# linnanwang/FastGen

Hardware: AMD Instinct MI355X
Metric: images/sec at 4-step distilled (DMD2) sampling (higher is better)
Workload: dtype fp32 (tensors, accumulate) with split-bf16 x3 MFMA conv products; 1 GPU; EDM CIFAR-10 32x32 SongUNet (55.7M params) DMD2 4-step 'sde' sampling, batch=512 per GPU; global_batch=512, sample_steps=4, parallelism=replicas x1 (no data-path collective), graph=True

## Files before the change

### fastgen_amd/csrc/conv.h

```cpp
#pragma once
#include <hip/hip_runtime.h>

struct ConvArgs {
    const void* src1;
    const void* src2;
    int C1, C2;
    int Hs, Ws;
    int H, W;
    int B;
    const float2* ab;
    const void* wpack;
    const void* wpack_ws;
    const float* bias;
    const float* temb;
    int temb_stride;
    const void* resid;
    float scale;
    void* out;
    int Cout;
    float2* stats;
    int dbg;
    void* q_out;
    void* k_out;
    void* vt_out;
    const float* gate = nullptr;
    int gate_stride = 0;
    int act = 0;
    int heads = 0, head_dim = 0;
    size_t heads_lo_off = 0;
};

enum { PRO_NONE = 0, PRO_GN = 1, PRO_GN_SILU = 2 };
enum { RES_NONE = 0, RES_DOWN = 1, RES_UP = 2 };
enum { OUT_NHWC = 0, OUT_QKV = 1, OUT_TOK = 2, OUT_HEADS = 3 };

int launch_conv_fused(int dtype, int ks, int pro, int res, int outmode, const ConvArgs& a, hipStream_t stream);
int conv_stat_slots(int W);
bool conv_ws_supported(int dtype, int ks, int pro, int res, int outmode, const ConvArgs& a);
bool conv_ws_enabled();
int launch_conv_ws(int res, const ConvArgs& a, hipStream_t stream, bool prepare_only, int pro = PRO_GN_SILU);
bool conv_ws_shape_ok(int dtype, int cout, int cin, int res);
int launch_pack_conv_weights_ws(const float* w_oihw, void* wpack_ws, int cout, int cin, hipStream_t stream);
bool conv_x3ws_supported(int ks, int pro, int res, int outmode, const ConvArgs& a);
bool conv_x3ws_shape_ok(int cout, int cin, int res);
int conv_x3ws_stat_slots(int W);
int launch_conv_x3ws(int res, const ConvArgs& a, hipStream_t stream, bool prepare_only, int pro = PRO_GN_SILU);
int launch_pack_conv_weights_x3ws(const float* w_oihw, void* wpack_ws, int cout, int cin, hipStream_t stream);
int conv_launch_stat_slots(int dtype, int ks, int pro, int res, int outmode, const ConvArgs& a);
int launch_conv_ws_debug(const ConvArgs& a, int abl, hipStream_t stream);
int launch_conv_debug(int dtype, const ConvArgs& a, hipStream_t stream);
int conv_prepare_all(int dtype);
size_t conv_pack_elems(int cout, int cin, int ks);
int launch_pack_conv_weights(int dtype, const float* w_oihw, void* wpack, int cout, int cin, int ks, int qkv_perm,
                             hipStream_t stream);
```

### fastgen_amd/csrc/conv.hip

```cpp
#include "common.h"
#include "conv.h"
#include <stdlib.h>

#include <type_traits>

namespace {

constexpr int PITCH = 144;
constexpr int NTHR = 256;

template <int KS, int LOGW>
struct Geom {
    static constexpr int W = 1 << LOGW;
    static constexpr int LOGTW = (LOGW == 5) ? 4 : LOGW;
    static constexpr int TW = 1 << LOGTW;
    static constexpr int LOGTH = 3;
    static constexpr int TH = 1 << LOGTH;
    static constexpr int IMGS = 128 / (TH * TW);
    static constexpr int TCOLS = W / TW;
    static constexpr int TPI = (IMGS > 1) ? 1 : (W / TH) * TCOLS;
    static constexpr int PAD = KS / 2;
    static constexpr int HW_ = TW + 2 * PAD;
    static constexpr int HH_ = TH + 2 * PAD;
    static constexpr int HALO_PIX = IMGS * HH_ * HW_;
// ... 427 lines not shown
                for (int i4 = 0; i4 < 16; i4 += 4) {
                    const int p = mt * 32 + acc_row(i4, h);
                    const int x = col0 + (p & (G::TW - 1));
                    const int y = row0 + ((p >> G::LOGTW) & (G::TH - 1));
                    const int n = n_base + (p >> (G::LOGTW + G::LOGTH));
                    if (n < a.B)
                    {
                        const size_t vo = ((size_t)n * (OUTMODE == OUT_HEADS ? a.heads * a.head_dim : 256) + cl) * HWo + y * G::W + x;
                        const f32x4 vv = {acc[mt][nt][i4] + bias, acc[mt][nt][i4 + 1] + bias, acc[mt][nt][i4 + 2] + bias,
                                          acc[mt][nt][i4 + 3] + bias};
                        if constexpr (OUTMODE == OUT_HEADS && std::is_same<T, bf16x3>::value)
                            store4_split(reinterpret_cast<__bf16*>(vt) + vo, a.heads_lo_off, vv);
                        else
                            store4(vt + vo, vv);
                    }
                }
            }
        }
    }
}

template <typename T>
__global__ void pack_conv_weights_kernel(const float* __restrict__ w, typename DT<T>::WT* __restrict__ out, int cout, int cin, int ks,
                                         int qkv_perm) {
    constexpr int KC = DT<T>::KC, KK = KC / 16, WP = DT<T>::WPARTS;
    const int taps = ks * ks;
    const size_t total = (size_t)cout * cin * taps;
    for (size_t idx = (size_t)blockIdx.x * blockDim.x + threadIdx.x; idx < total; idx += (size_t)gridDim.x * blockDim.x) {
        size_t t = idx;
        const int j = t % 8; t /= 8;
        const int lane = t % 64; t /= 64;
        const int kk = t % KK; t /= KK;
        const int tap = t % taps; t /= taps;
        const int nchunk = cin / KC;
        const int chunk = t % nchunk; t /= nchunk;
        const int nt = (int)t;
        int co = nt * 32 + (lane & 31);
        if (qkv_perm) {
            const int C = cout / 3;
            co = (co % C) * 3 + co / C;
        }
        const int ci = chunk * KC + kk * 16 + 8 * (lane >> 5) + j;
        const float v = w[((size_t)co * cin + ci) * taps + tap];
        if constexpr (WP == 1) {
            out[idx] = (typename DT<T>::WT)v;
        } else {
            const size_t o = (idx / 512) * 1024 + (idx % 512);
            const __bf16 hi = (__bf16)v;
            out[o] = hi;
            out[o + 512] = (__bf16)(v - (float)hi);
        }
    }
}

size_t g_debug_extra_lds = 0;
bool g_prepare_only = false;

template <typename T, int KS, int PRO, int RES, int LOGW, int OUTMODE, int ABL = 0>
int launch_one(const ConvArgs& a, hipStream_t stream) {
    using G = Geom<KS, LOGW>;
    const int tiles = (G::IMGS > 1) ? (a.B + G::IMGS - 1) / G::IMGS : a.B * G::TPI;
    const size_t lds = 2 * (size_t)G::ABUF + (ABL ? g_debug_extra_lds : 0);
    auto kern = conv_fused_kernel<T, KS, PRO, RES, LOGW, OUTMODE, ABL>;
    static bool attr_done[16] = {};
    const int dev = fg_device_slot();
    if (dev < 0) return (int)hipErrorInvalidDevice;
    if (!attr_done[dev] || (ABL && g_debug_extra_lds)) {
        hipError_t e = hipFuncSetAttribute(reinterpret_cast<const void*>(kern), hipFuncAttributeMaxDynamicSharedMemorySize, (int)lds);
        if (e != hipSuccess) return (int)e;
        attr_done[dev] = true;
    }
    if (g_prepare_only) return 0;
    constexpr int NCOL = 128 * conv_nt(KS, LOGW, OUTMODE);
    dim3 grid(tiles, (a.Cout + NCOL - 1) / NCOL);
    hipLaunchKernelGGL(kern, grid, dim3(NTHR), lds, stream, a);
    return (int)hipGetLastError();
}

template <typename T, int KS, int PRO, int RES, int OUTMODE>
int launch_w(const ConvArgs& a, hipStream_t s) {
    switch (a.W) {
        case 32: return launch_one<T, KS, PRO, RES, 5, OUTMODE>(a, s);
        case 16: return launch_one<T, KS, PRO, RES, 4, OUTMODE>(a, s);
        case 8: return launch_one<T, KS, PRO, RES, 3, OUTMODE>(a, s);
    }
    return (int)hipErrorInvalidValue;
}

template <typename T>
int launch_t(int ks, int pro, int res, int outmode, const ConvArgs& a, hipStream_t s) {
    if (outmode == OUT_QKV) {
        if (ks == 1 && pro == PRO_GN && res == RES_NONE) return launch_w<T, 1, PRO_GN, RES_NONE, OUT_QKV>(a, s);
        return (int)hipErrorInvalidValue;
    }
    if (outmode == OUT_TOK || outmode == OUT_HEADS) {
        if (ks != 1 || pro != PRO_NONE || res != RES_NONE || a.W != 16) return (int)hipErrorInvalidValue;
        return outmode == OUT_TOK ? launch_one<T, 1, PRO_NONE, RES_NONE, 4, OUT_TOK>(a, s) : launch_one<T, 1, PRO_NONE, RES_NONE, 4, OUT_HEADS>(a, s);
    }
    if (ks == 3 && pro == PRO_GN_SILU) {
        if (res == RES_NONE) return launch_w<T, 3, PRO_GN_SILU, RES_NONE, OUT_NHWC>(a, s);
        if (res == RES_UP) return launch_w<T, 3, PRO_GN_SILU, RES_UP, OUT_NHWC>(a, s);
    }
    if (ks == 3 && pro == PRO_NONE && res == RES_NONE) return launch_w<T, 3, PRO_NONE, RES_NONE, OUT_NHWC>(a, s);
    if (ks == 1 && pro == PRO_NONE) {
        if (res == RES_NONE) return launch_w<T, 1, PRO_NONE, RES_NONE, OUT_NHWC>(a, s);
        if (res == RES_DOWN) return launch_w<T, 1, PRO_NONE, RES_DOWN, OUT_NHWC>(a, s);
        if (res == RES_UP) return launch_w<T, 1, PRO_NONE, RES_UP, OUT_NHWC>(a, s);
    }
    return (int)hipErrorInvalidValue;
}

int dispatch_t(int dtype, int ks, int pro, int res, int outmode, const ConvArgs& a, hipStream_t s) {
    switch (dtype) {
        case 0: return launch_t<float>(ks, pro, res, outmode, a, s);
        case 1: return launch_t<__bf16>(ks, pro, res, outmode, a, s);
        case 2: return launch_t<bf16x3>(ks, pro, res, outmode, a, s);
    }
    return (int)hipErrorInvalidValue;
}

}

int launch_conv_debug(int dtype, const ConvArgs& a, hipStream_t stream) {
    if (dtype != 1 || a.W != 32) return (int)hipErrorInvalidValue;
    g_debug_extra_lds = (a.dbg & 16) ? 48 * 1024 : 0;
    switch (a.dbg & 15) {
        case 0: return launch_one<__bf16, 3, PRO_GN_SILU, RES_NONE, 5, OUT_NHWC, 0>(a, stream);
        case 1: return launch_one<__bf16, 3, PRO_GN_SILU, RES_NONE, 5, OUT_NHWC, 1>(a, stream);
        case 2: return launch_one<__bf16, 3, PRO_GN_SILU, RES_NONE, 5, OUT_NHWC, 2>(a, stream);
        case 3: return launch_one<__bf16, 3, PRO_GN_SILU, RES_NONE, 5, OUT_NHWC, 3>(a, stream);
        case 4: return launch_one<__bf16, 3, PRO_GN_SILU, RES_NONE, 5, OUT_NHWC, 4>(a, stream);
        case 5: return launch_one<__bf16, 3, PRO_GN_SILU, RES_NONE, 5, OUT_NHWC, 5>(a, stream);
        case 6: return launch_one<__bf16, 3, PRO_GN_SILU, RES_NONE, 5, OUT_NHWC, 6>(a, stream);
        case 7: return launch_one<__bf16, 3, PRO_GN_SILU, RES_NONE, 5, OUT_NHWC, 7>(a, stream);
    }
    return (int)hipErrorInvalidValue;
}

int launch_conv_fused(int dtype, int ks, int pro, int res, int outmode, const ConvArgs& a, hipStream_t stream) {
    const int kc = dtype == 1 ? DT<__bf16>::KC : DT<float>::KC;
    if (a.H != a.W || (a.W != 8 && a.W != 16 && a.W != 32)) return (int)hipErrorInvalidValue;
    const bool tok = outmode == OUT_TOK || outmode == OUT_HEADS;
    if ((a.C1 % kc) || (a.C2 % kc) || (a.Cout % (tok ? 64 : 256)) || a.B <= 0) return (int)hipErrorInvalidValue;
    if (outmode == OUT_HEADS && (a.heads <= 0 || (a.head_dim % 4) || a.Cout != 3 * a.heads * a.head_dim || ((a.heads * a.head_dim) % 64) ||
                                 !a.q_out || !a.k_out || !a.vt_out))
        return (int)hipErrorInvalidValue;
    if (res == RES_NONE && (a.Hs != a.H || a.Ws != a.W)) return (int)hipErrorInvalidValue;
    if (res == RES_DOWN && (a.Hs != 2 * a.H || a.Ws != 2 * a.W)) return (int)hipErrorInvalidValue;
    if (res == RES_UP && (2 * a.Hs != a.H || 2 * a.Ws != a.W)) return (int)hipErrorInvalidValue;
    if (pro != PRO_NONE && !a.ab) return (int)hipErrorInvalidValue;
    if (outmode == OUT_QKV && (a.Cout != 768 || a.W > 16)) return (int)hipErrorInvalidValue;
    if (conv_ws_enabled() && conv_ws_supported(dtype, ks, pro, res, outmode, a)) return launch_conv_ws(res, a, stream, false, pro);
    if (dtype == 2 && conv_ws_enabled() && conv_x3ws_supported(ks, pro, res, outmode, a)) return launch_conv_x3ws(res, a, stream, false, pro);
    return dispatch_t(dtype, ks, pro, res, outmode, a, stream);
}

bool conv_ws_enabled() {
    static const bool on = [] {
        const char* e = getenv("FASTGEN_AMD_CONV_WS");
        return !(e && e[0] == '0');
    }();
    return on;
}

int conv_launch_stat_slots(int dtype, int ks, int pro, int res, int outmode, const ConvArgs& a) {
    if (dtype == 2 && conv_ws_enabled() && conv_x3ws_supported(ks, pro, res, outmode, a)) return conv_x3ws_stat_slots(a.W);
    return conv_stat_slots(a.W);
}

int conv_stat_slots(int W) { return W == 32 ? Geom<3, 5>::TPI : (W == 16 ? Geom<3, 4>::TPI : Geom<3, 3>::TPI); }

int conv_prepare_all(int dtype) {
    g_prepare_only = true;
    int rc = 0;
    ConvArgs a{};
    a.B = 1;
    a.Cout = 256;
    const int ws[3] = {8, 16, 32};
    for (int wi = 0; wi < 3 && !rc; ++wi) {
        a.W = a.H = ws[wi];
        for (int res = 0; res < 3 && !rc; ++res) {
            if (res != RES_DOWN)
                rc = dispatch_t(dtype, 3, PRO_GN_SILU, res, OUT_NHWC, a, nullptr);
            if (!rc) rc = dispatch_t(dtype, 1, PRO_NONE, res, OUT_NHWC, a, nullptr);
        }
        if (!rc) rc = dispatch_t(dtype, 3, PRO_NONE, RES_NONE, OUT_NHWC, a, nullptr);
        if (!rc && a.W <= 16) rc = dispatch_t(dtype, 1, PRO_GN, RES_NONE, OUT_QKV, a, nullptr);
        if (!rc && a.W == 16) rc = dispatch_t(dtype, 1, PRO_NONE, RES_NONE, OUT_TOK, a, nullptr);
        if (!rc && a.W == 16) rc = dispatch_t(dtype, 1, PRO_NONE, RES_NONE, OUT_HEADS, a, nullptr);
    }
    g_prepare_only = false;
    if (!rc && dtype == 2) {
        ConvArgs w{};
        for (int res : {RES_NONE, RES_UP})
            for (int ww : {32, 16, 8}) {
                if (ww == 8 && res != RES_NONE) continue;
                w.W = w.H = ww;
                if (!rc) rc = launch_conv_x3ws(res, w, nullptr, true, PRO_GN_SILU);
                if (!rc && res == RES_NONE) rc = launch_conv_x3ws(res, w, nullptr, true, PRO_NONE);
            }
    }
    if (!rc && dtype == 1) {
        ConvArgs w{};
        for (int res : {RES_NONE, RES_UP}) {
            w.W = w.H = 32;
            if (!rc) rc = launch_conv_ws(res, w, nullptr, true);
            if (res == RES_NONE) {
                w.C1 = -128;
                if (!rc) rc = launch_conv_ws(res, w, nullptr, true);
                w.C1 = 0;
            }
            w.W = w.H = 16;
            if (!rc) rc = launch_conv_ws(res, w, nullptr, true);
        }
    }
    return rc;
}

size_t conv_pack_elems(int cout, int cin, int ks) { return (size_t)cout * cin * ks * ks; }

int launch_pack_conv_weights(int dtype, const float* w, void* out, int cout, int cin, int ks, int qkv_perm,
                             hipStream_t stream) {
    const size_t total = conv_pack_elems(cout, cin, ks);
    const int grid = (int)((total + 255) / 256 < 4096 ? (total + 255) / 256 : 4096);
    if (dtype == 1)
        hipLaunchKernelGGL(pack_conv_weights_kernel<__bf16>, dim3(grid), dim3(256), 0, stream, w, (__bf16*)out, cout, cin, ks, qkv_perm);
    else if (dtype == 2)
        hipLaunchKernelGGL(pack_conv_weights_kernel<bf16x3>, dim3(grid), dim3(256), 0, stream, w, (__bf16*)out, cout, cin, ks, qkv_perm);
    else
        hipLaunchKernelGGL(pack_conv_weights_kernel<float>, dim3(grid), dim3(256), 0, stream, w, (float*)out, cout, cin, ks, qkv_perm);
    return (int)hipGetLastError();
}
```

### fastgen_amd/csrc/engine.hip

```cpp
#include <hip/hip_runtime.h>

#include <cmath>
#include <cstdarg>
#include <cstdio>
#include <cstdlib>
#include <cstring>
#include <string>
#include <map>
#include <vector>

#include "../../include/fastgen_amd.h"
#include "common.h"
#include "adm.h"
#include "edm2.h"
#include "conv.h"
#include "misc.h"

namespace {

thread_local std::string g_err;

int fail(int code, const char* fmt, ...) {
    char buf[512];
    va_list ap;
// ... 554 lines not shown
            n.w = h->add(n.key + ".weight", {cout});
            n.b = h->add(n.key + ".bias", {cout});
            h->dec.push_back(n);
            Block a;
            a.key = "model.dec." + res_name(res) + "_aux_conv";
            a.kind = K_AUX_CONV;
            a.cin = cout;
            a.cout = c.img_channels;
            a.res_in = a.res_out = res;
            a.w = h->add(a.key + ".weight", {a.cout, a.cin, 3, 3});
            a.b = h->add(a.key + ".bias", {a.cout});
            h->dec.push_back(a);
        }
    }
    h->add("model.logvar_linear.weight", {1, h->noise_ch});
    h->add("model.logvar_linear.bias", {1});
    for (auto& b : h->enc)
        if (b.kind == K_BLOCK) h->blocks.push_back(&b);
    for (auto& b : h->dec)
        if (b.kind == K_BLOCK) h->blocks.push_back(&b);
}

int check_supported(const fg_edm* h) {
    const fg_edm_config& c = h->cfg;
    const int kc = h->dtype ? 64 : 32;
    if (c.img_resolution != 32 && c.img_resolution != 16 && c.img_resolution != 8)
        return fail(FG_EINVAL, "img_resolution %d unsupported (8, 16, 32)", c.img_resolution);
    if ((c.img_resolution >> (c.num_levels - 1)) < 8)
        return fail(FG_EINVAL, "lowest resolution %d < 8 unsupported", c.img_resolution >> (c.num_levels - 1));
    if (c.img_channels > 4) return fail(FG_EINVAL, "img_channels %d > 4 unsupported", c.img_channels);
    for (const Block* b : h->blocks) {
        if (b->cout != 256) return fail(FG_EINVAL, "%s: out_channels %d unsupported (kernels are tiled for 256)", b->key.c_str(), b->cout);
        if (b->cin % kc || (b->cin - b->skip_c) % kc)
            return fail(FG_EINVAL, "%s: in_channels %d not a multiple of %d", b->key.c_str(), b->cin, kc);
        if (b->attn && b->res_out > 16) return fail(FG_EINVAL, "%s: attention at %dx%d unsupported", b->key.c_str(), b->res_out, b->res_out);
    }
    return FG_OK;
}

void adm_build_layout(fg_edm* h);
int adm_check_supported(const fg_edm* h);
size_t adm_plan_workspace(const fg_edm* h, int B, Arena& A, Workspace& w);
int adm_pack_weights(fg_edm* h, hipStream_t s);
int adm_forward(fg_edm* h, const float* x_t, const double* t, int t_stride, const float* labels, float* out, int B, Workspace& w,
                hipStream_t s);
int adm_refuse(const fg_edm* h, const char* what) {
    return fail(FG_EINVAL, "%s is not implemented for DhariwalUNet (forward and sampling only)", what);
}

size_t plan_workspace(const fg_edm* h, int B, Arena& A, Workspace& w) {
    if (h->adm) return adm_plan_workspace(h, B, A, w);
    const fg_edm_config& c = h->cfg;
    const size_t tsz = h->dtype ? 2 : 4;
    const int R = c.img_resolution;
    size_t max_act = 0;
    int max_c = 0, max_attn_hw = 0;
    for (const Block& b : h->enc) max_act = std::max(max_act, (size_t)b.res_out * b.res_out * b.cout);
    for (const Block* b : h->blocks) {
        max_act = std::max(max_act, (size_t)b->res_out * b->res_out * b->cout);
        max_c = std::max(max_c, std::max(b->cin, b->cout));
        if (b->attn) max_attn_hw = std::max(max_attn_hw, b->res_out * b->res_out);
    }
    w.coef = A.get<float>(5 * (size_t)B);
    w.emb0 = A.get<float>((size_t)B * h->cond_ch);
    w.emb1 = A.get<float>((size_t)B * h->emb_ch);
    w.emb = A.get<float>((size_t)B * h->emb_ch);
    w.temb = A.get<float>((size_t)B * h->temb_total);
    w.ab0 = A.get<float2>((size_t)B * max_c);
    w.ab1 = A.get<float2>((size_t)B * max_c);
    w.ab2 = A.get<float2>((size_t)B * max_c);
    const size_t st_elems = (size_t)B * 32 * 64;
    auto act = [&](size_t elems, size_t st_n) {
        Act a;
        a.p = A.take(elems * tsz);
        a.st = A.get<float2>(st_n);
        return a;
    };
    w.skip.clear();
    for (const Block& b : h->enc)
        w.skip.push_back(act((size_t)B * b.res_out * b.res_out * b.cout,
                             (b.kind == K_STEM && b.p_stem) ? (size_t)B * b.res_out * b.res_out : st_elems));
    w.xa = act((size_t)B * max_act, st_elems);
    w.xb = act((size_t)B * max_act, st_elems);
    w.h = act((size_t)B * max_act, st_elems);
    w.sbuf = A.take((size_t)B * max_act * tsz);
    w.pool = A.take((size_t)B * max_act * tsz);
    w.cvt1 = A.take((size_t)B * max_act * 4 * tsz);
    w.cvt2 = A.take((size_t)B * max_act * 4 * tsz);
    w.xattn = act((size_t)B * max_attn_hw * 256, st_elems);
    w.aout = A.take((size_t)B * max_attn_hw * 256 * tsz);
    w.q = A.take((size_t)B * max_attn_hw * 256 * tsz);
    w.k = A.take((size_t)B * max_attn_hw * 256 * tsz);
    w.vt = A.take((size_t)B * max_attn_hw * 256 * tsz);
    const size_t img = (size_t)B * c.img_channels * R * R;
    w.x = A.get<float>(img);
    w.x_pred = A.get<float>(img);
    w.eps = A.get<float>(img);
    w.tl = A.get<double>(ScalarRing::kDoubles);
    w.seed = A.get<uint64_t>(8);
    return (A.off + 255) & ~(size_t)255;
}

int conv_launch(fg_edm* h, int ks, int pro, int res, int outmode, const ConvArgs& a, hipStream_t s) {
    const bool timed = h->prof_on && ks == 3 && res == RES_NONE && a.W == 32 && outmode == OUT_NHWC;
    hipEvent_t e0 = nullptr, e1 = nullptr;
    if (timed) {
        if (hipEventCreate(&e0) != hipSuccess || hipEventCreate(&e1) != hipSuccess) return (int)hipErrorUnknown;
        (void)hipEventRecord(e0, s);
    }
    const int rc = launch_conv_fused(h->cmode, ks, pro, res, outmode, a, s);
    if (timed) {
        (void)hipEventRecord(e1, s);
        h->prof_ev.push_back(e0);
        h->prof_ev.push_back(e1);
        h->prof_flops += 2.0 * a.B * a.H * a.W * (double)a.Cout * 9.0 * (a.C1 + a.C2);
    }
    return rc;
}

const float kSkipScale = (float)std::sqrt(0.5);
const float kBlockEps = 1e-6f;

int norm_coeffs(int dtype, const Act& x1, int c1, const Act& x2, int c2, const float* gamma, const float* beta, float2* ab,
                int B, int hw, hipStream_t s, float2* mr = nullptr) {
    if (x1.st && (!c2 || x2.st))
        HIP_TRY(launch_gn_finalize(x1.st, c1, x1.slots, c2 ? x2.st : nullptr, c2, c2 ? x2.slots : 0, gamma, beta, kBlockEps, ab, B, hw, s, mr));
    else
        HIP_TRY(launch_gn_coeffs(dtype, x1.p, c1, c2 ? x2.p : nullptr, c2, gamma, beta, kBlockEps, ab, B, hw, s, mr));
    return FG_OK;
}

void use_stash(Workspace& w, const BlockStash& st) {
    w.h.p = st.h;
    w.ab0 = st.ab0, w.ab1 = st.ab1, w.mr0 = st.mr0, w.mr1 = st.mr1;
    w.a1d = st.a1d;
    w.drop.block = st.index;
    if (st.xattn) {
        w.xattn.p = st.xattn;
        w.ab2 = st.ab2, w.mr2 = st.mr2;
        w.q = st.q, w.k = st.k, w.vt = st.vt, w.aout = st.aout;
    }
}
int block_index(const fg_edm* h, const Block* b) {
    for (size_t i = 0; i < h->blocks.size(); ++i)
        if (h->blocks[i] == b) return (int)i;
    return -1;
}

int run_block(fg_edm* h, const Block& b, const Act& x1, int c1, const Act& x2, int c2, const float* temb, Act& out, int B,
              Workspace& w, hipStream_t s) {
    if (c1 + c2 != b.cin) return fail(FG_EINVAL, "%s: got %d+%d input channels, expected %d", b.key.c_str(), c1, c2, b.cin);
    const int hw_in = b.res_in * b.res_in, hw = b.res_out * b.res_out;
    const int res_mode = b.down ? RES_DOWN : (b.up ? RES_UP : RES_NONE);
    const int slots = conv_stat_slots(b.res_out);
    int rc;
    if ((rc = norm_coeffs(h->dtype, x1, c1, x2, c2, h->P(b.norm0_w), h->P(b.norm0_b), w.ab0, B, hw_in, s, w.mr0))) return rc;
    ConvArgs a{};
    a.src1 = x1.p; a.src2 = c2 ? x2.p : nullptr; a.C1 = c1; a.C2 = c2;
    a.Hs = a.Ws = b.res_in; a.H = a.W = b.res_out; a.B = B;
    a.ab = w.ab0; a.wpack = b.p_conv0; a.wpack_ws = b.p_conv0_ws; a.bias = h->P(b.conv0_b);
    a.temb = temb + b.temb_off; a.temb_stride = h->temb_total;
    a.resid = nullptr; a.scale = 1.0f; a.out = w.h.p; a.Cout = b.cout; a.stats = w.h.st;
    if (b.down && !c2) {
        HIP_TRY(launch_gn_silu_pool(h->dtype, x1.p, w.ab0, w.pool, B, b.res_out, b.res_out, c1, s));
        a.src1 = w.pool; a.Hs = a.Ws = b.res_out; a.ab = nullptr;
        w.h.slots = conv_launch_stat_slots(h->cmode, 3, PRO_NONE, RES_NONE, OUT_NHWC, a);
        HIP_TRY(conv_launch(h, 3, PRO_NONE, RES_NONE, OUT_NHWC, a, s));
    } else {
        w.h.slots = conv_launch_stat_slots(h->cmode, 3, PRO_GN_SILU, res_mode, OUT_NHWC, a);
        HIP_TRY(conv_launch(h, 3, PRO_GN_SILU, res_mode, OUT_NHWC, a, s));
    }
    const void* resid = x1.p;
    if (b.has_skip) {
        ConvArgs k{};
        k.src1 = x1.p; k.src2 = c2 ? x2.p : nullptr; k.C1 = c1; k.C2 = c2;
        k.Hs = k.Ws = b.res_in; k.H = k.W = b.res_out; k.B = B;
        k.wpack = b.p_skip; k.bias = h->P(b.skip_b); k.scale = 1.0f; k.out = w.sbuf; k.Cout = b.cout;
        HIP_TRY(conv_launch(h, 1, PRO_NONE, res_mode, OUT_NHWC, k, s));
        resid = w.sbuf;
    }
    HIP_TRY(launch_gn_finalize(w.h.st, b.cout, w.h.slots, nullptr, 0, 0, h->P(b.norm1_w), h->P(b.norm1_b), kBlockEps, w.ab1, B, hw, s, w.mr1));
    Act& x_mid = b.attn ? w.xattn : out;
    ConvArgs d{};
    d.src1 = w.h.p; d.C1 = b.cout; d.Hs = d.Ws = d.H = d.W = b.res_out; d.B = B;
    d.ab = w.ab1; d.wpack = b.p_conv1; d.wpack_ws = b.p_conv1_ws; d.bias = h->P(b.conv1_b);
    d.resid = resid; d.scale = kSkipScale; d.out = x_mid.p; d.Cout = b.cout; d.stats = x_mid.st;
    if (w.a1d) {
        HIP_TRY(launch_gn_act(h->dtype, 0, w.h.p, b.cout, nullptr, 0, w.ab1, w.a1d, B, b.res_out, 0, s, w.drop));
        d.src1 = w.a1d; d.ab = nullptr;
        x_mid.slots = conv_launch_stat_slots(h->cmode, 3, PRO_NONE, RES_NONE, OUT_NHWC, d);
        HIP_TRY(conv_launch(h, 3, PRO_NONE, RES_NONE, OUT_NHWC, d, s));
    } else {
        x_mid.slots = conv_launch_stat_slots(h->cmode, 3, PRO_GN_SILU, RES_NONE, OUT_NHWC, d);
        HIP_TRY(conv_launch(h, 3, PRO_GN_SILU, RES_NONE, OUT_NHWC, d, s));
    }
    if (b.attn) {
        HIP_TRY(launch_gn_finalize(x_mid.st, b.cout, x_mid.slots, nullptr, 0, 0, h->P(b.norm2_w), h->P(b.norm2_b), kBlockEps, w.ab2, B, hw, s, w.mr2));
        ConvArgs q{};
        q.src1 = x_mid.p; q.C1 = b.cout; q.Hs = q.Ws = q.H = q.W = b.res_out; q.B = B;
        q.ab = w.ab2; q.wpack = b.p_qkv; q.bias = b.qkv_bias; q.scale = 1.0f; q.Cout = 3 * b.cout;
        q.q_out = w.q; q.k_out = w.k; q.vt_out = w.vt;
        HIP_TRY(conv_launch(h, 1, PRO_GN, RES_NONE, OUT_QKV, q, s));
        HIP_TRY(launch_attention(h->cmode, w.q, w.k, w.vt, w.aout, B, hw, s));
        ConvArgs p{};
        p.src1 = w.aout; p.C1 = b.cout; p.Hs = p.Ws = p.H = p.W = b.res_out; p.B = B;
        p.wpack = b.p_proj; p.bias = h->P(b.proj_b); p.resid = x_mid.p; p.scale = kSkipScale; p.out = out.p; p.Cout = b.cout;
        p.stats = out.st;
        HIP_TRY(conv_launch(h, 1, PRO_NONE, RES_NONE, OUT_NHWC, p, s));
        out.slots = slots;
    }
    return FG_OK;
}

int run_mapping(fg_edm* h, const float* labels, int B, Workspace& w, hipStream_t s) {
    const fg_edm_config& c = h->cfg;
    HIP_TRY(launch_mapping_in(w.coef + B, w.coef + 4 * (size_t)B, h->freqs, labels, c.label_dim,
                              h->P(h->find("model.map_label.weight")), h->P(h->find("model.map_label.bias")), w.emb0, B,
                              h->cond_ch, h->noise_ch, s, h->augment, h->augment ? h->P(h->find("model.map_augment.weight")) : nullptr, c.augment_dim));
    HIP_TRY(launch_linear(w.emb0, h->P(h->find("model.map_layer0.weight")), h->P(h->find("model.map_layer0.bias")), w.emb1,
                          B, h->cond_ch, h->emb_ch, 1, s));
    HIP_TRY(launch_linear(w.emb1, h->P(h->find("model.map_layer1.weight")), h->P(h->find("model.map_layer1.bias")), w.emb, B,
                          h->emb_ch, h->emb_ch, 1, s));
    HIP_TRY(launch_linear(w.emb, h->aff_w, h->aff_b, w.temb, B, h->emb_ch, h->temb_total, 0, s));
    return FG_OK;
}

int run_forward(fg_edm* h, const float* x_t, const double* t, int t_stride, const double* r, int r_stride,
                const float* labels, float* out, int B, Workspace& w, hipStream_t s, float* const* feats = nullptr,
                bool early = false, TrainStash* ts = nullptr) {
    if (h->adm) return adm_forward(h, x_t, t, t_stride, labels, out, B, w, s);
    const fg_edm_config& c = h->cfg;
    HIP_TRY(launch_precond_coef(t, t_stride, c.r_timestep ? r : nullptr, r_stride, c.sigma_data, h->shift(), 1e-6,
                                c.drop_precond, w.coef, B, s));
    int rc = run_mapping(h, labels, B, w, s);
    if (rc) return rc;
    w.drop = DropArgs{};
    if (ts && h->dropout_p > 0.f) w.drop.p = h->dropout_p, w.drop.seed = h->dropout_seed;
    const Act none;
    const Act* x = nullptr;
    for (size_t i = 0; i < h->enc.size(); ++i) {
        const Block& b = h->enc[i];
        if (b.kind == K_STEM) {
            if (b.p_stem) {
                HIP_TRY(launch_stem(h->dtype, x_t, w.coef, b.p_stem, h->P(b.b), w.skip[i].p, w.skip[i].st, B, b.res_out, b.cin, s));
                w.skip[i].slots = b.res_out * b.res_out / 32;
            } else {
                HIP_TRY(launch_conv_in(h->dtype, x_t, w.coef, h->P(b.w), h->P(b.b), w.skip[i].p, B, b.res_out, b.cin, b.cout, s));
                w.skip[i].st = nullptr;
            }
        } else {
            if (ts) use_stash(w, ts->blocks[block_index(h, &b)]);
            rc = run_block(h, b, *x, b.cin, none, 0, w.temb, w.skip[i], B, w, s);
            if (rc) return rc;
            if (feats && b.tap >= 0 && feats[b.tap])
                HIP_TRY(launch_act_to_nchw(h->dtype, w.skip[i].p, feats[b.tap], B, b.cout, b.res_out * b.res_out, s));
        }
        x = &w.skip[i];
    }
    if (early) return FG_OK;
    int sp = (int)h->enc.size();
    Act* pong[2] = {&w.xa, &w.xb};
    int cur = 0;
    size_t di = 0;
    const float2* aux_ab = nullptr;
    for (const Block& b : h->dec) {
        if (b.kind == K_BLOCK) {
            const Act& x2 = b.skip_c ? w.skip[--sp] : none;
            Act& dst = ts ? ts->dec_store[di++] : *pong[cur];
            if (ts) use_stash(w, ts->blocks[block_index(h, &b)]);
            rc = run_block(h, b, *x, b.cin - b.skip_c, x2, b.skip_c, w.temb, dst, B, w, s);
            if (rc) return rc;
            x = &dst;
            cur ^= 1;
        } else if (b.kind == K_AUX_NORM) {
            if (ts) w.ab0 = ts->aux_ab, w.mr0 = ts->aux_mr;
            if ((rc = norm_coeffs(h->dtype, *x, b.cin, none, 0, h->P(b.w), h->P(b.b), w.ab0, B, b.res_in * b.res_in, s, ts ? w.mr0 : nullptr))) return rc;
            aux_ab = w.ab0;
        } else if (b.kind == K_AUX_CONV) {
            if (b.p_aux)
                HIP_TRY(launch_aux_head(h->cmode, x->p, aux_ab, b.p_aux, h->P(b.b), x_t, w.coef, out, B, b.cin, b.cout, s, ts ? ts->raw_out : nullptr));
            else
                HIP_TRY(launch_aux_out(h->dtype, x->p, aux_ab, h->P(b.w), h->P(b.b), x_t, w.coef, out, B, b.res_out, b.cin, b.cout, s, ts ? ts->raw_out : nullptr));
        }
    }
    return FG_OK;
}

int enqueue_sampler(fg_edm* h, const float* noise, const float* labels, const double* t_list, int steps, int type,
                    int loop, const float* eps, float* out, int B, Workspace& w, hipStream_t s) {
    const fg_edm_config& c = h->cfg;
    const int64_t total = (int64_t)B * c.img_channels * c.img_resolution * c.img_resolution;
    const StudentLoop L{noise, t_list, steps, type, c.schedule, total, w.x, w.eps, eps, w.tl, w.seed, out, s};
    if (loop == FG_LOOP_MEANFLOW)
        return meanflow_loop(L, w.x_pred, [&](int i, float* u) {
            return run_forward(h, w.x, w.tl + i, 0, w.tl + (type == FG_SAMPLE_SDE ? steps : i + 1), 0, labels, u, B, w, s);
        });
    return x0_loop(L, w.x_pred, [&](int i, float* pred) { return run_forward(h, w.x, w.tl + i, 0, w.tl + steps, 0, labels, pred, B, w, s); });
}

int ensure_device_state(fg_edm* h) {
    if (h->device_ready) return FG_OK;
    int rc;
    const size_t tsz = h->dtype ? 2 : 4;
    for (Block* b : h->blocks) {
        if ((rc = h->alloc(&b->p_conv0, conv_pack_elems(b->cout, b->cin, 3) * tsz))) return rc;
        if ((rc = h->alloc(&b->p_conv1, conv_pack_elems(b->cout, b->cout, 3) * tsz))) return rc;
        const bool x3 = h->cmode == FG_DTYPE_BF16X3;
        if ((x3 ? conv_x3ws_shape_ok(b->cout, b->cin, b->res_out) : conv_ws_shape_ok(h->cmode, b->cout, b->cin, b->res_out)) && !b->down &&
            (rc = h->alloc(&b->p_conv0_ws, conv_pack_elems(b->cout, b->cin, 3) * tsz)))
            return rc;
        if ((x3 ? conv_x3ws_shape_ok(b->cout, b->cout, b->res_out) : conv_ws_shape_ok(h->cmode, b->cout, b->cout, b->res_out)) &&
            (rc = h->alloc(&b->p_conv1_ws, conv_pack_elems(b->cout, b->cout, 3) * tsz)))
            return rc;
        if (b->has_skip && (rc = h->alloc(&b->p_skip, conv_pack_elems(b->cout, b->cin, 1) * tsz))) return rc;
        if (b->attn) {
            if ((rc = h->alloc(&b->p_qkv, conv_pack_elems(3 * b->cout, b->cout, 1) * tsz))) return rc;
            if ((rc = h->alloc(&b->p_proj, conv_pack_elems(b->cout, b->cout, 1) * tsz))) return rc;
            if ((rc = h->alloc((void**)&b->qkv_bias, sizeof(float) * 3 * b->cout))) return rc;
        }
    }
    for (Block& b : h->enc)
        if (b.kind == K_STEM && stem_supported(b.res_out, b.cin, b.cout))
            if ((rc = h->alloc(&b.p_stem, stem_pack_elems() * tsz))) return rc;
    for (Block& b : h->dec)
        if (b.kind == K_AUX_CONV && aux_head_supported(h->cmode, b.res_out, b.cin, b.cout))
            if ((rc = h->alloc(&b.p_aux, aux_pack_elems(b.cin) * tsz))) return rc;
    if ((rc = h->alloc((void**)&h->aff_w, sizeof(float) * (size_t)h->temb_total * h->emb_ch))) return rc;
    if ((rc = h->alloc((void**)&h->aff_b, sizeof(float) * (size_t)h->temb_total))) return rc;
    const int half = h->noise_ch / 2;
    std::vector<float> fr(half);
    for (int j = 0; j < half; ++j) fr[j] = powf(1.0f / 10000.0f, (float)j / (float)(half - 1));
    if ((rc = h->alloc((void**)&h->freqs, sizeof(float) * half))) return rc;
    HIP_TRY(hipMemcpy(h->freqs, fr.data(), sizeof(float) * half, hipMemcpyHostToDevice));
    if (conv_prepare_all(h->cmode) != 0) return fail(FG_EHIP, "hipFuncSetAttribute(dynamic LDS) failed");
    if (launch_attention(h->cmode, nullptr, nullptr, nullptr, nullptr, 1, 256, nullptr) != 0) return fail(FG_EHIP, "attention prepare failed");
    h->device_ready = true;
    return FG_OK;
}

#include "engine_adm.inc"

}

extern "C" {

const char* fg_last_error(void) { return g_err.c_str(); }
const char* fg_version(void) { return "fastgen_amd 0.1 gfx950"; }

int fg_edm_create(const fg_edm_config* cfg, fg_edm** out) {
    if (!cfg || !out) return fail(FG_EINVAL, "null argument");
    if (cfg->num_levels < 1 || cfg->num_levels > FG_MAX_LEVELS || cfg->num_attn_resolutions < 0 ||
        cfg->num_attn_resolutions > FG_MAX_LEVELS)
        return fail(FG_EINVAL, "bad num_levels / num_attn_resolutions");
    if (cfg->compute_dtype != FG_DTYPE_F32 && cfg->compute_dtype != FG_DTYPE_BF16 && cfg->compute_dtype != FG_DTYPE_BF16X3)
        return fail(FG_EINVAL, "bad compute_dtype");
    if ((cfg->drop_precond & ~3) || (cfg->schedule != FG_SCHEDULE_EDM && cfg->schedule != FG_SCHEDULE_RF) ||
        (cfg->r_timestep & ~1))
        return fail(FG_EINVAL, "bad r_timestep / drop_precond / schedule");
    if (cfg->model_channels <= 0 || cfg->model_channels % 16 || cfg->channel_mult_noise < 1 || cfg->channel_mult_emb < 1)
        return fail(FG_EINVAL, "bad channel configuration");
    if (cfg->model_type != FG_MODEL_SONGUNET && cfg->model_type != FG_MODEL_DHARIWAL) return fail(FG_EINVAL, "bad model_type");
    fg_edm* h = new fg_edm();
// ... 623 lines not shown
```

Measured before the change: 2719 img/s.

## Add warp-specialized streaming 1x1 conv kernel for split-bf16 x3 skip convs

Adds a new persistent 512-thread 1x1 convolution kernel for the x3 split-bf16 mode. Four producer waves load fp32 activations through a register ring, split them into hi/lo bf16 and write double-buffered LDS. Four consumer waves keep weight fragments in registers and run MFMAs plus a fused bias/temb/stat epilogue. It is enabled only for skip and proj 1x1 convs with no residual, Cin >= 512 and W of 32 or 8, so it mostly hits the concatenated-input skip convs in the decoder. The aim is to overlap global loads with the MFMA work of these convs, at the cost of a new code path and extra LDS and register use.

Measured after the change: 2720 img/s (median of 4 runs). Within noise of the previous version (+0.0%).

```diff
diff --git a/fastgen_amd/csrc/conv.h b/fastgen_amd/csrc/conv.h
--- a/fastgen_amd/csrc/conv.h
+++ b/fastgen_amd/csrc/conv.h
@@ -28,6 +28,7 @@
     int act = 0;
     int heads = 0, head_dim = 0;
     size_t heads_lo_off = 0;
+    bool stream1x1 = false;
 };
 
 enum { PRO_NONE = 0, PRO_GN = 1, PRO_GN_SILU = 2 };
@@ -46,6 +47,10 @@
 int conv_x3ws_stat_slots(int W);
 int launch_conv_x3ws(int res, const ConvArgs& a, hipStream_t stream, bool prepare_only, int pro = PRO_GN_SILU);
 int launch_pack_conv_weights_x3ws(const float* w_oihw, void* wpack_ws, int cout, int cin, hipStream_t stream);
+bool conv1_x3_supported(int dtype, int ks, int pro, int res, int outmode, const ConvArgs& a);
+bool conv1_x3_enabled();
+int conv1_x3_stat_slots(int W);
+int launch_conv1_x3(int res, const ConvArgs& a, hipStream_t stream, bool prepare_only);
 int conv_launch_stat_slots(int dtype, int ks, int pro, int res, int outmode, const ConvArgs& a);
 int launch_conv_ws_debug(const ConvArgs& a, int abl, hipStream_t stream);
 int launch_conv_debug(int dtype, const ConvArgs& a, hipStream_t stream);
diff --git a/fastgen_amd/csrc/conv.hip b/fastgen_amd/csrc/conv.hip
--- a/fastgen_amd/csrc/conv.hip
+++ b/fastgen_amd/csrc/conv.hip
@@ -603,6 +603,7 @@
     if (outmode == OUT_QKV && (a.Cout != 768 || a.W > 16)) return (int)hipErrorInvalidValue;
     if (conv_ws_enabled() && conv_ws_supported(dtype, ks, pro, res, outmode, a)) return launch_conv_ws(res, a, stream, false, pro);
     if (dtype == 2 && conv_ws_enabled() && conv_x3ws_supported(ks, pro, res, outmode, a)) return launch_conv_x3ws(res, a, stream, false, pro);
+    if (conv1_x3_supported(dtype, ks, pro, res, outmode, a)) return launch_conv1_x3(res, a, stream, false);
     return dispatch_t(dtype, ks, pro, res, outmode, a, stream);
 }
 
@@ -616,6 +617,7 @@
 
 int conv_launch_stat_slots(int dtype, int ks, int pro, int res, int outmode, const ConvArgs& a) {
     if (dtype == 2 && conv_ws_enabled() && conv_x3ws_supported(ks, pro, res, outmode, a)) return conv_x3ws_stat_slots(a.W);
+    if (conv1_x3_supported(dtype, ks, pro, res, outmode, a)) return conv1_x3_stat_slots(a.W);
     return conv_stat_slots(a.W);
 }
 
@@ -651,6 +653,15 @@
                 if (!rc && res == RES_NONE) rc = launch_conv_x3ws(res, w, nullptr, true, PRO_NONE);
             }
     }
+    if (!rc && dtype == 2) {
+        ConvArgs w{};
+        for (int res : {RES_NONE, RES_UP})
+            for (int ww : {32, 16, 8}) {
+                if (ww == 8 && res != RES_NONE) continue;
+                w.W = w.H = ww;
+                if (!rc) rc = launch_conv1_x3(res, w, nullptr, true);
+            }
+    }
     if (!rc && dtype == 1) {
         ConvArgs w{};
         for (int res : {RES_NONE, RES_UP}) {
diff --git a/fastgen_amd/csrc/conv1_x3.hip b/fastgen_amd/csrc/conv1_x3.hip
--- /dev/null
+++ b/fastgen_amd/csrc/conv1_x3.hip
@@ -0,0 +1,332 @@
+#include "common.h"
+#include "conv.h"
+#include <stdlib.h>
+
+namespace {
+
+constexpr int C1_NTHR = 512;
+constexpr int C1_KC = 32;
+constexpr int C1_DEPTH = 6;
+constexpr int C1_PITCH = 144;
+constexpr int C1_ABUF = 128 * C1_PITCH;
+constexpr int C1_EP_PITCH = 64 * 4 + 16;
+constexpr int C1_EP = 32 * C1_EP_PITCH;
+constexpr int C1_LDS = 2 * C1_ABUF + 4 * C1_EP;
+constexpr int C1_STEPW = 2 * 512 * 2;
+
+template <int LOGW>
+struct C1Geom {
+    static constexpr int W = 1 << LOGW;
+    static constexpr int LOGTW = (LOGW == 5) ? 4 : LOGW;
+    static constexpr int TW = 1 << LOGTW;
+    static constexpr int LOGTH = 3;
+    static constexpr int TH = 8;
+    static constexpr int IMGS = 128 / (TH * TW);
+    static constexpr int TCOLS = W / TW;
+    static constexpr int TPI = (IMGS > 1) ? 1 : (W / TH) * TCOLS;
+};
+
+__device__ __forceinline__ void c1_barrier() {
+    asm volatile("s_waitcnt lgkmcnt(0)\n\ts_barrier" ::: "memory");
+}
+
+template <int RES, int LOGW>
+__global__ __launch_bounds__(C1_NTHR) void conv1_x3_kernel(const ConvArgs a, const int ntiles) {
+    using G = C1Geom<LOGW>;
+    using F = Frag8<bf16x3>;
+    extern __shared__ __attribute__((aligned(16))) char smem[];
+
+    const int tid = threadIdx.x;
+    const int lane = tid & 63;
+    const int wave = __builtin_amdgcn_readfirstlane(tid >> 6);
+    const int Cin = a.C1 + a.C2;
+    const int nchunk = Cin / C1_KC;
+    const int G8 = (int)gridDim.x >> 3;
+    const int wg = ((gridDim.x & 7) == 0) ? ((int)blockIdx.x & 7) * G8 + ((int)blockIdx.x >> 3) : (int)blockIdx.x;
+    const int gstride = (int)gridDim.x;
+    const int my_tiles = (ntiles - wg + gstride - 1) / gstride;
+    const int S = my_tiles * nchunk;
+    const int H = a.H;
+
+    auto tile_coord = [&](int t, int& n_base, int& slot, int& row0, int& col0) {
+        n_base = (G::IMGS > 1) ? t * G::IMGS : t / G::TPI;
+        slot = (G::IMGS > 1) ? 0 : t % G::TPI;
+        row0 = (slot / G::TCOLS) * G::TH;
+        col0 = (slot % G::TCOLS) * G::TW;
+    };
+
+    if (wave < 4) {
+        const int r = lane & 31, h = lane >> 5;
+        const int wst = nchunk * C1_STEPW;
+        const __amdgpu_buffer_rsrc_t wrs = make_rsrc(reinterpret_cast<const __bf16*>(a.wpack) + (size_t)(wave * 2) * wst);
+        const int wlane = lane * 8;
+        F bfr[2][2];
+#pragma unroll
+        for (int nt = 0; nt < 2; ++nt)
+#pragma unroll
+            for (int kk = 0; kk < 2; ++kk) load_frag_rsrc(bfr[nt][kk], wrs, wlane, nt * wst + kk * 1024);
+
+        f32x16 acc[4][2];
+#pragma unroll
+        for (int mt = 0; mt < 4; ++mt)
+#pragma unroll
+            for (int nt = 0; nt < 2; ++nt)
+#pragma unroll
+                for (int i = 0; i < 16; ++i) acc[mt][nt][i] = 0.f;
+
+        const int lane_off = r * C1_PITCH + h * 16;
+        char* const ep = smem + 2 * C1_ABUF + wave * C1_EP;
+        float* const out = reinterpret_cast<float*>(a.out);
+        const float* const resid = reinterpret_cast<const float*>(a.resid);
+
+        constexpr int QPW = 16, RP = 4, NP = 8;
+        constexpr int MT_PER_IMG = 4 / G::IMGS;
+        const int c4 = lane % QPW, prow = lane / QPW;
+        const int co0 = wave * 64 + c4 * 4;
+        auto epilogue = [&](int tile) __attribute__((always_inline)) {
+            int n_base, slot, row0, col0;
+            tile_coord(tile, n_base, slot, row0, col0);
+            f32x4 bias4 = {0.f, 0.f, 0.f, 0.f};
+            if (a.bias) bias4 = *reinterpret_cast<const f32x4*>(a.bias + co0);
+            float ssum[G::IMGS], ssq[G::IMGS];
+#pragma unroll
+            for (int im = 0; im < G::IMGS; ++im) ssum[im] = ssq[im] = 0.f;
+            auto goff = [&](int mt, int j, bool& ok) -> size_t {
+                const int p = mt * 32 + j * RP + prow;
+                const int x = col0 + (p & (G::TW - 1));
+                const int y = row0 + ((p >> G::LOGTW) & (G::TH - 1));
+                const int n = n_base + mt / MT_PER_IMG;
+                ok = n < a.B;
+                return (((size_t)n * H + y) * G::W + x) * 256 + co0;
+            };
+            f32x4 rcur[NP], rnext[NP];
+            auto issue_resid = [&](int mt, f32x4 (&rr)[NP]) {
+#pragma unroll
+                for (int j = 0; j < NP; ++j) {
+                    bool ok;
+                    const size_t go = goff(mt, j, ok);
+                    rr[j] = f32x4{0.f, 0.f, 0.f, 0.f};
+                    if (ok) rr[j] = *reinterpret_cast<const f32x4*>(resid + go);
+                }
+            };
+            if (resid) issue_resid(0, rcur);
+#pragma unroll
+            for (int mt = 0; mt < 4; ++mt) {
+                const int im = mt / MT_PER_IMG;
+                const int n = n_base + im;
+                if (resid && mt + 1 < 4) issue_resid(mt + 1, rnext);
+#pragma unroll
+                for (int nt = 0; nt < 2; ++nt)
+#pragma unroll
+                    for (int i = 0; i < 16; ++i) {
+                        *reinterpret_cast<float*>(ep + acc_row(i, h) * C1_EP_PITCH + (nt * 32 + r) * 4) = acc[mt][nt][i];
+                        acc[mt][nt][i] = 0.f;
+                    }
+                f32x4 add = bias4;
+                if (a.temb && n < a.B) add += *reinterpret_cast<const f32x4*>(a.temb + (size_t)n * a.temb_stride + co0);
+#pragma unroll
+                for (int j = 0; j < NP; ++j) {
+                    const int pl = j * RP + prow;
+                    f32x4 v = *reinterpret_cast<const f32x4*>(ep + pl * C1_EP_PITCH + c4 * 16);
+                    bool ok;
+                    const size_t go = goff(mt, j, ok);
+                    if (ok) {
+                        v += add;
+                        if (resid) v += rcur[j];
+                        v *= a.scale;
+                        *reinterpret_cast<f32x4*>(out + go) = v;
+                        ssum[im] += (v[0] + v[1]) + (v[2] + v[3]);
+                        ssq[im] += (v[0] * v[0] + v[1] * v[1]) + (v[2] * v[2] + v[3] * v[3]);
+                    }
+                }
+#pragma unroll
+                for (int j = 0; j < NP; ++j) rcur[j] = rnext[j];
+            }
+            if (a.stats) {
+#pragma unroll
+                for (int im = 0; im < G::IMGS; ++im) {
+                    float sv = ssum[im], qv = ssq[im];
+#pragma unroll
+                    for (int sh = QPW; sh < 64; sh <<= 1) {
+                        sv += __shfl_xor(sv, sh);
+                        qv += __shfl_xor(qv, sh);
+                    }
+                    const int n = n_base + im;
+                    if (prow == 0 && n < a.B) a.stats[((size_t)n * G::TPI + slot) * 64 + (co0 >> 2)] = make_float2(sv, qv);
+                }
+            }
+        };
+
+        c1_barrier();
+        int c = 0, tile = wg;
+        for (int g = 0; g < S; ++g) {
+            const char* abase = smem + (g & 1) * C1_ABUF + lane_off;
+            const int cn = (c + 1 == nchunk) ? 0 : c + 1;
+            const int pnext = cn * C1_STEPW;
+            F a0[4], a1[4];
+#pragma unroll
+            for (int mt = 0; mt < 4; ++mt) a0[mt] = lds_read_a<bf16x3>(abase + mt * (32 * C1_PITCH), 0);
+#pragma unroll
+            for (int mt = 0; mt < 4; ++mt) a1[mt] = lds_read_a<bf16x3>(abase + mt * (32 * C1_PITCH), 1);
+            auto mma8 = [&](int kk, const F (&af)[4]) {
+#pragma unroll
+                for (int mt = 0; mt < 4; ++mt)
+#pragma unroll
+                    for (int nt = 0; nt < 2; ++nt) mma16(acc[mt][nt], af[mt], bfr[nt][kk]);
+#pragma unroll
+                for (int nt = 0; nt < 2; ++nt) load_frag_rsrc(bfr[nt][kk], wrs, wlane, pnext + nt * wst + kk * 1024);
+            };
+            __builtin_amdgcn_sched_barrier(0);
+            mma8(0, a0);
+            __builtin_amdgcn_sched_barrier(0);
+            mma8(1, a1);
+            __builtin_amdgcn_sched_barrier(0);
+            if (cn == 0) {
+                epilogue(tile);
+                tile += gstride;
+            }
+            c = cn;
+            c1_barrier();
+        }
+        return;
+    }
+
+    const int ptid = tid - 256;
+    const int oct = ptid & 3;
+    const int q0 = ptid >> 2;
+    const char* const src1 = reinterpret_cast<const char*>(a.src1);
+    const char* const src2 = reinterpret_cast<const char*>(a.src2);
+    struct Raw {
+        f32x4 v[2][2];
+    };
+    Raw raw[C1_DEPTH];
+    unsigned off1[2], off2[2];
+    int lt = wg, lc = 0;
+    auto tile_setup = [&](int t) __attribute__((always_inline)) {
+        int n_base, slot, row0, col0;
+        tile_coord(t, n_base, slot, row0, col0);
+#pragma unroll
+        for (int i = 0; i < 2; ++i) {
+            const int p = q0 + 64 * i;
+            const int x = col0 + (p & (G::TW - 1));
+            const int y = row0 + ((p >> G::LOGTW) & (G::TH - 1));
+            const int n = min(n_base + (p >> (G::LOGTW + G::LOGTH)), a.B - 1);
+            const int sy = (RES == RES_UP) ? (y >> 1) : y, sx = (RES == RES_UP) ? (x >> 1) : x;
+            const unsigned pix = (unsigned)((n * a.Hs + sy) * a.Ws + sx);
+            off1[i] = (pix * (unsigned)a.C1 + oct * 8) * 4u;
+            off2[i] = (pix * (unsigned)a.C2 + oct * 8) * 4u;
+        }
+    };
+    auto load = [&](Raw& rw) __attribute__((always_inline)) {
+        if (lc == 0) tile_setup(lt);
+        const bool first = lc * C1_KC < a.C1;
+        const char* base = first ? src1 + lc * (C1_KC * 4) : src2 + (lc * C1_KC - a.C1) * 4;
+#pragma unroll
+        for (int i = 0; i < 2; ++i) {
+            const char* p = base + (first ? off1[i] : off2[i]);
+            rw.v[i][0] = *reinterpret_cast<const f32x4*>(p);
+            rw.v[i][1] = *reinterpret_cast<const f32x4*>(p + 16);
+        }
+        if (++lc == nchunk) {
+            lc = 0;
+            lt += gstride;
+        }
+    };
+    auto store = [&](const Raw& rw, char* abuf) __attribute__((always_inline)) {
+#pragma unroll
+        for (int i = 0; i < 2; ++i) {
+            float v[8];
+#pragma unroll
+            for (int j = 0; j < 8; ++j) v[j] = rw.v[i][j >> 2][j & 3];
+            bf16x8 hi, lo;
+            split8(v, hi, lo);
+            char* p = abuf + (q0 + 64 * i) * C1_PITCH + oct * 16;
+            *reinterpret_cast<bf16x8*>(p) = hi;
+            *reinterpret_cast<bf16x8*>(p + 64) = lo;
+        }
+    };
+
+#pragma unroll
+    for (int j = 0; j < C1_DEPTH; ++j)
+        if (j < S) load(raw[j]);
+    store(raw[0], smem);
+    if (C1_DEPTH < S) load(raw[0]);
+    c1_barrier();
+    for (int g0 = 0; g0 < S; g0 += C1_DEPTH) {
+#pragma unroll
+        for (int j = 0; j < C1_DEPTH; ++j) {
+            const int g = g0 + j;
+            if (g < S) {
+                if (g + 1 < S) {
+                    store(raw[(j + 1) % C1_DEPTH], smem + ((g + 1) & 1) * C1_ABUF);
+                    if (g + 1 + C1_DEPTH < S) load(raw[(j + 1) % C1_DEPTH]);
+                }
+                c1_barrier();
+            }
+        }
+    }
+}
+
+int g_c1_cus[16] = {};
+
+template <int RES, int LOGW>
+int launch_c1_one(const ConvArgs& a, hipStream_t stream, bool prepare_only) {
+    using G = C1Geom<LOGW>;
+    auto kern = conv1_x3_kernel<RES, LOGW>;
+    const int dev = fg_device_slot();
+    if (dev < 0) return (int)hipErrorInvalidDevice;
+    static bool attr_done[16] = {};
+    if (!attr_done[dev]) {
+        hipError_t e = hipFuncSetAttribute(reinterpret_cast<const void*>(kern), hipFuncAttributeMaxDynamicSharedMemorySize, C1_LDS);
+        if (e != hipSuccess) return (int)e;
+        attr_done[dev] = true;
+    }
+    if (!g_c1_cus[dev]) {
+        int n = 0;
+        if (hipDeviceGetAttribute(&n, hipDeviceAttributeMultiprocessorCount, dev) != hipSuccess || n <= 0) return (int)hipErrorUnknown;
+        g_c1_cus[dev] = n;
+    }
+    if (prepare_only) return 0;
+    const int ntiles = (G::IMGS > 1) ? (a.B + G::IMGS - 1) / G::IMGS : a.B * G::TPI;
+    const int grid = ntiles < g_c1_cus[dev] ? ntiles : g_c1_cus[dev];
+    hipLaunchKernelGGL(kern, dim3(grid), dim3(C1_NTHR), C1_LDS, stream, a, ntiles);
+    return (int)hipGetLastError();
+}
+
+}
+
+bool conv1_x3_enabled() {
+    static const bool on = [] {
+        const char* e = getenv("FASTGEN_AMD_CONV1X1");
+        return !(e && e[0] == '0');
+    }();
+    return on;
+}
+
+int conv1_x3_stat_slots(int W) { return W == 32 ? C1Geom<5>::TPI : (W == 16 ? C1Geom<4>::TPI : C1Geom<3>::TPI); }
+
+bool conv1_x3_supported(int dtype, int ks, int pro, int res, int outmode, const ConvArgs& a) {
+    if (!a.stream1x1 || !conv1_x3_enabled()) return false;
+    if (dtype != 2 || ks != 1 || pro != PRO_NONE || outmode != OUT_NHWC || a.Cout != 256 || a.B <= 0) return false;
+    if (a.H != a.W || (a.W != 8 && a.W != 16 && a.W != 32)) return false;
+    if ((a.C1 % C1_KC) || (a.C2 % C1_KC) || a.C1 <= 0 || a.C2 < 0 || !a.wpack || !a.out || a.gate || a.act) return false;
+    const size_t src_bytes = (size_t)a.B * a.Hs * a.Ws * (size_t)(a.C1 > a.C2 ? a.C1 : a.C2) * 4;
+    if (src_bytes >= (1ull << 32)) return false;
+    if (res != RES_NONE || a.Hs != a.H || a.Ws != a.W) return false;
+    return !a.resid && a.C1 + a.C2 >= 512 && (a.W == 32 || a.W == 8);
+}
+
+int launch_conv1_x3(int res, const ConvArgs& a, hipStream_t stream, bool prepare_only) {
+    if (res == RES_UP) {
+        if (a.W == 32) return launch_c1_one<RES_UP, 5>(a, stream, prepare_only);
+        if (a.W == 16) return launch_c1_one<RES_UP, 4>(a, stream, prepare_only);
+        return (int)hipErrorInvalidValue;
+    }
+    if (res != RES_NONE) return (int)hipErrorInvalidValue;
+    switch (a.W) {
+        case 32: return launch_c1_one<RES_NONE, 5>(a, stream, prepare_only);
+        case 16: return launch_c1_one<RES_NONE, 4>(a, stream, prepare_only);
+        case 8: return launch_c1_one<RES_NONE, 3>(a, stream, prepare_only);
+    }
+    return (int)hipErrorInvalidValue;
+}
diff --git a/fastgen_amd/csrc/engine.hip b/fastgen_amd/csrc/engine.hip
--- a/fastgen_amd/csrc/engine.hip
+++ b/fastgen_amd/csrc/engine.hip
@@ -730,7 +730,6 @@
     if (c1 + c2 != b.cin) return fail(FG_EINVAL, "%s: got %d+%d input channels, expected %d", b.key.c_str(), c1, c2, b.cin);
     const int hw_in = b.res_in * b.res_in, hw = b.res_out * b.res_out;
     const int res_mode = b.down ? RES_DOWN : (b.up ? RES_UP : RES_NONE);
-    const int slots = conv_stat_slots(b.res_out);
     int rc;
     if ((rc = norm_coeffs(h->dtype, x1, c1, x2, c2, h->P(b.norm0_w), h->P(b.norm0_b), w.ab0, B, hw_in, s, w.mr0))) return rc;
     ConvArgs a{};
@@ -754,6 +753,7 @@
         k.src1 = x1.p; k.src2 = c2 ? x2.p : nullptr; k.C1 = c1; k.C2 = c2;
         k.Hs = k.Ws = b.res_in; k.H = k.W = b.res_out; k.B = B;
         k.wpack = b.p_skip; k.bias = h->P(b.skip_b); k.scale = 1.0f; k.out = w.sbuf; k.Cout = b.cout;
+        k.stream1x1 = !w.a1d;
         HIP_TRY(conv_launch(h, 1, PRO_NONE, res_mode, OUT_NHWC, k, s));
         resid = w.sbuf;
     }
@@ -784,8 +784,9 @@
         p.src1 = w.aout; p.C1 = b.cout; p.Hs = p.Ws = p.H = p.W = b.res_out; p.B = B;
         p.wpack = b.p_proj; p.bias = h->P(b.proj_b); p.resid = x_mid.p; p.scale = kSkipScale; p.out = out.p; p.Cout = b.cout;
         p.stats = out.st;
+        p.stream1x1 = !w.a1d;
+        out.slots = conv_launch_stat_slots(h->cmode, 1, PRO_NONE, RES_NONE, OUT_NHWC, p);
         HIP_TRY(conv_launch(h, 1, PRO_NONE, RES_NONE, OUT_NHWC, p, s));
-        out.slots = slots;
     }
     return FG_OK;
 }
```
